# samuel-vitorino/sopro

Measured on NVIDIA H100. Metric: ar_frames_per_sec, higher is better.
Workload: dtype f32 math / bf16 weight storage

## Files before the change

### include/sopro_b200.h

```cpp
#ifndef SOPRO_B200_H_
#define SOPRO_B200_H_

#include <stddef.h>
#include <stdint.h>

#ifdef __cplusplus
extern "C" {
#endif

#define SOPRO_MAX_AR_LAYERS 16

enum sopro_status {
  SOPRO_OK = 0,
  SOPRO_ERR_INVALID = -1,
  SOPRO_ERR_CUDA = -2,
  SOPRO_ERR_UNSUPPORTED = -3,
  SOPRO_ERR_STATE = -4
};

enum sopro_wdtype { SOPRO_W_F32 = 0, SOPRO_W_BF16 = 1 };

typedef struct sopro_ar_config {
  int32_t d_model;
  int32_t n_layers;
// ... 64 lines not shown
int sopro_ar_session_create(sopro_engine_t* e, int max_batch, int max_steps, int max_text_len,
                            sopro_ar_session_t** out);
int sopro_ar_session_destroy(sopro_ar_session_t* s);

int sopro_ar_session_set_team(sopro_ar_session_t* s, int utts_per_team);

int sopro_ar_begin(sopro_ar_session_t* s, int batch, int steps, const float* cond_ar,
                   const float* txt_seq, int text_stride, const int32_t* text_len,
                   const float* noise, int noise_k, const sopro_ar_sampling_t* sampling,
                   void* stream);

int sopro_ar_run(sopro_ar_session_t* s, int n_steps, void* stream);

int sopro_ar_outputs(sopro_ar_session_t* s, const int32_t** tokens, const int32_t** n_tokens,
                     const int32_t** done);
int sopro_ar_read(sopro_ar_session_t* s, int32_t* tokens_host, int32_t* n_tokens_host,
                  int32_t* done_host, void* stream);
int sopro_ar_position(sopro_ar_session_t* s);

int sopro_ar_generate_host(sopro_ar_session_t* s, int batch, int steps, const float* cond_ar,
                           const float* txt_seq, int text_stride, const int32_t* text_len,
                           const float* noise, int noise_k, const sopro_ar_sampling_t* sampling,
                           int32_t* tokens_out, int32_t* n_tokens_out, void* stream);

typedef struct sopro_noise sopro_noise_t;
int sopro_noise_create(uint64_t seed, sopro_noise_t** out);
int sopro_noise_rows(sopro_noise_t* g, int n_rows, int vocab, int keep, float* out);
int sopro_noise_destroy(sopro_noise_t* g);

int sopro_ar_set_forced_tokens(sopro_ar_session_t* s, const int32_t* forced);
int sopro_ar_set_trace(sopro_ar_session_t* s, float* trace_blocks, float* trace_logits);
int sopro_ar_set_timing(sopro_ar_session_t* s, int64_t* buf, int step);
int sopro_ar_set_attn_trace(sopro_ar_session_t* s, float* probs, int64_t ld);
int sopro_ar_debug_sampled(sopro_ar_session_t* s, int32_t* dst, void* stream);
int sopro_ar_debug_kv(sopro_ar_session_t* s, float* k_dst, float* v_dst, void* stream);
int sopro_debug_pack_w6(const float* W, int N, int K, uint16_t* out);
int sopro_debug_sample(const float* logits, int vocab, const int32_t* hist, int n_hist, const float* noise, int noise_k,
                       const sopro_ar_sampling_t* sampling, int recovery, int device, int32_t* token_out);


#define SOPRO_MIMI_MAX_LAYERS 16
#define SOPRO_MIMI_MAX_RATIOS 8

typedef struct sopro_mimi_config {
  int32_t hidden;
  int32_t codebook_dim;
  int32_t n_q;
  int32_t n_sem;
  int32_t vocab;
  int32_t n_layers;
  int32_t n_heads;
  int32_t ffn;
  int32_t window;
  int32_t num_filters;
  int32_t kernel;
  int32_t last_kernel;
  int32_t res_kernel;
  int32_t compress;
  int32_t n_ratios;
  int32_t ratios[SOPRO_MIMI_MAX_RATIOS];
  float norm_eps;
  float rope_theta;
} sopro_mimi_config_t;

typedef struct sopro_mimi_layer_weights {
  const float *ln1_w, *ln1_b;
// ... 318 lines not shown
```

### sopro_b200/_lib.py

```python
from __future__ import annotations

import ctypes as C
import math
import os
from typing import List, Optional, Sequence

import torch

MAX_AR_LAYERS = 16
_HERE = os.path.dirname(os.path.abspath(__file__))
LIB_PATH = os.path.join(_HERE, "lib", "libsopro_b200.so")


class SoproError(RuntimeError):
    pass


class ArConfig(C.Structure):
    _fields_ = [
        ("d_model", C.c_int32), ("n_layers", C.c_int32), ("kernel", C.c_int32), ("n_heads", C.c_int32),
        ("vocab", C.c_int32), ("eos_id", C.c_int32),
        ("dilation", C.c_int32 * MAX_AR_LAYERS), ("has_attn", C.c_int32 * MAX_AR_LAYERS),
        ("weight_dtype", C.c_int32),
    ]
# ... 103 lines not shown

class RefPrepKvLayer(C.Structure):
    _fields_ = [(n, C.POINTER(C.c_float)) for n in ("nkv_w", "k_w", "v_w")]


class RefPrepWeights(C.Structure):
    _fields_ = [(n, C.POINTER(C.c_float)) for n in ("sv_emb", "sv_cb_weights", "sv_dw0_w", "sv_dw0_b", "sv_dw1_w", "sv_dw1_b",
                                                    "pool_w0", "pool_b0", "pool_w2")] + [("pool_b2", C.c_float)] + [
        (n, C.POINTER(C.c_float)) for n in ("proj_w", "proj_b", "cb_embed", "ref_cb_weights")] + [
        ("ref_block", SsmBlockWeights * 16), ("ref_norm_w", C.POINTER(C.c_float)), ("layer", RefPrepKvLayer * 8)]


_VP, _I, _I32P = C.c_void_p, C.c_int, C.POINTER(C.c_int32)
SYMBOLS = {
    "sopro_last_error": (C.c_char_p, []),
    "sopro_version": (C.c_char_p, []),
    "sopro_engine_create": (_I, [C.POINTER(ArConfig), C.POINTER(ArWeights), _I, C.POINTER(_VP)]),
    "sopro_engine_destroy": (_I, [_VP]),
    "sopro_engine_step_weight_bytes": (C.c_int64, [_VP]),
    "sopro_engine_num_sms": (_I, [_VP]),
    "sopro_ar_session_create": (_I, [_VP, _I, _I, _I, C.POINTER(_VP)]),
    "sopro_ar_session_destroy": (_I, [_VP]),
    "sopro_ar_session_set_team": (_I, [_VP, _I]),
    "sopro_ar_begin": (_I, [_VP, _I, _I, _VP, _VP, _I, _I32P, _VP, _I, C.POINTER(ArSampling), _VP]),
    "sopro_ar_run": (_I, [_VP, _I, _VP]),
    "sopro_ar_outputs": (_I, [_VP, C.POINTER(_VP), C.POINTER(_VP), C.POINTER(_VP)]),
    "sopro_ar_read": (_I, [_VP, _VP, _VP, _VP, _VP]),
    "sopro_ar_position": (_I, [_VP]),
    "sopro_ar_generate_host": (_I, [_VP, _I, _I, _VP, _VP, _I, _I32P, _VP, _I, C.POINTER(ArSampling), _VP, _VP, _VP]),
    "sopro_ar_set_forced_tokens": (_I, [_VP, _VP]),
    "sopro_ar_set_trace": (_I, [_VP, _VP, _VP]),
    "sopro_ar_set_timing": (_I, [_VP, _VP, _I]),
    "sopro_ar_set_attn_trace": (_I, [_VP, _VP, C.c_int64]),
    "sopro_ar_debug_sampled": (_I, [_VP, _VP, _VP]),
    "sopro_ar_debug_kv": (_I, [_VP, _VP, _VP, _VP]),
    "sopro_noise_create": (_I, [C.c_uint64, _VP]),
    "sopro_noise_rows": (_I, [_VP, _I, _I, _I, _VP]),
    "sopro_noise_destroy": (_I, [_VP]),
    "sopro_debug_pack_w6": (_I, [_VP, _I, _I, _VP]),
    "sopro_debug_sample": (_I, [_VP, _I, _VP, _I, _VP, _I, _VP, _I, _I, _VP]),
    "sopro_mimi_create": (_I, [C.POINTER(MimiConfigC), C.POINTER(MimiWeights), _I, C.POINTER(_VP)]),
    "sopro_mimi_destroy": (_I, [_VP]),
    "sopro_mimi_samples_per_frame": (C.c_int64, [_VP]),
    "sopro_mimi_decode": (_I, [_VP, _VP, _I, _I, _VP, _VP]),
    "sopro_mimi_decode_host": (_I, [_VP, _VP, _I, _I, _VP, _VP]),
    "sopro_mimi_set_precision": (_I, [_VP, _I]),
    "sopro_mimi_set_graphs": (_I, [_VP, _I]),
    "sopro_mimi_check": (_I, [_VP, _VP]),
    "sopro_mimi_stream_create": (_I, [_VP, _I, C.POINTER(_VP)]),
    "sopro_mimi_stream_destroy": (_I, [_VP]),
    "sopro_mimi_stream_reset": (_I, [_VP, _VP]),
    "sopro_mimi_stream_frames": (C.c_int64, [_VP]),
    "sopro_mimi_decode_step": (_I, [_VP, _VP, _I, _VP, _VP]),
    "sopro_mimi_decode_step_host": (_I, [_VP, _VP, _I, _VP, _VP]),
    "sopro_mimi_encoder_create": (_I, [C.POINTER(MimiConfigC), C.POINTER(MimiEncoderWeights), _I, C.POINTER(_VP)]),
    "sopro_mimi_encoder_destroy": (_I, [_VP]),
    "sopro_mimi_encoded_frames": (C.c_int64, [_VP, C.c_int64]),
    "sopro_mimi_encode": (_I, [_VP, _VP, C.c_int64, _VP, _VP, _VP]),
    "sopro_mimi_encode_host": (_I, [_VP, _VP, C.c_int64, _VP, _VP, _VP]),
    "sopro_nar_create": (_I, [_VP, _VP, _I, C.POINTER(_VP)]),
    "sopro_nar_destroy": (_I, [_VP]),
    "sopro_nar_set_forced": (_I, [_VP, _VP]),
    "sopro_nar_set_contraction": (_I, [_VP, _I]),
    "sopro_nar_set_graphs": (_I, [_VP, _I]),
    "sopro_nar_set_trace": (_I, [_VP, _VP]),
    "sopro_debug_dense": (_I, [_VP, _VP, _VP, _VP, _VP, _VP, _VP, C.c_float, _I, _I, _I, _I, _I, _I, C.c_int64, C.c_int64,
# ... 185 lines not shown
```

### sopro_b200/csrc/ar_engine.cu

```cuda
#include <cuda_runtime.h>

#include <algorithm>
#include <cstdio>
#include <cstring>
#include <string>
#include <vector>

#include "../../include/sopro_b200.h"
#include "common.cuh"
#include "ar_kernel.cuh"

using namespace sopro;

namespace {

thread_local std::string g_err;

size_t align_up(size_t x, size_t a) { return (x + a - 1) / a * a; }

uint16_t f32_to_bf16_rne(float f) {
  uint32_t u;
  memcpy(&u, &f, 4);
  if ((u & 0x7fffffffu) > 0x7f800000u) return (uint16_t)((u >> 16) | 0x40);
  const uint32_t lsb = (u >> 16) & 1u;
// ... 23 lines not shown
};

}

namespace mimi {
void set_error(const char* msg) { g_err = msg; }
}

struct sopro_engine {
  int device = 0;
  int n_sms = 0;
  sopro_ar_config_t cfg{};
  int D = 0, F = 0, V = 0, Vpad = 0, H = 0, Dh = 0, Kc = 0, n_layers = 0, n_attn = 0;
  unsigned char* dev = nullptr;
  size_t dev_bytes = 0;
  int64_t step_weight_bytes = 0;
  LayerDev layer[kMaxLayers]{};
  const float* nkv_w[kMaxLayers]{};
  const void* wk[kMaxLayers]{};
  const void* wv[kMaxLayers]{};
  const float* final_norm_w = nullptr;
  const void* head_w = nullptr;
  const float* head_b = nullptr;
  const float* emb = nullptr;
  const float* epi[kMaxLayers]{};
  int KcP = 0, KcE = 0;
  long long ring_floats_per_utt = 0;
};

struct sopro_ar_session {
  sopro_engine* e = nullptr;
  int max_batch = 0, max_steps = 0, Lmax = 0;
  int utts_per_team = 0;
  float *ring = nullptr, *xa = nullptr, *xb = nullptr, *hbuf = nullptr, *qbuf = nullptr, *abuf = nullptr,
        *logits = nullptr, *kc = nullptr, *vc = nullptr;
  int *tokens = nullptr, *sampled = nullptr, *text_len = nullptr, *n_tokens = nullptr, *done = nullptr;
  UttState* st = nullptr;
  SamplingDev* samp = nullptr;
  unsigned* barrier = nullptr;
  unsigned* tok_ll = nullptr;
  unsigned seq_base = 0;
  TileDesc* tiles = nullptr;
  int* n_tiles = nullptr;
  unsigned char* stage_tiles = nullptr;
  std::vector<unsigned char> h_stage_tiles;
  int tile_P = -1, tile_wbuf = -1, tile_qatt = -1;
  bool qatt = false;
  std::vector<TileDesc> h_tiles;
  std::vector<int> h_ntiles;
  float *h_cond = nullptr, *h_txt = nullptr, *h_noise = nullptr;
  size_t h_cond_cap = 0, h_txt_cap = 0, h_noise_cap = 0;
  int B = 0, steps = 0, noise_k = 0, t_pos = 0;
  const float* cond = nullptr;
  const float* noise = nullptr;
  const int* forced = nullptr;
  float* trace_blocks = nullptr;
  float* trace_logits = nullptr;
  long long* timing = nullptr;
  int timing_step = -1;
  float* attn_trace = nullptr;
  int64_t attn_ld = 0;
  int max_len = 0;
  bool begun = false;
  std::vector<UttState> host_st;
  unsigned char* pin = nullptr;
  size_t pin_bytes = 0;
// ... 246 lines not shown
  A((void**)&s->n_tokens, B * 4);
  A((void**)&s->done, B * 4);
  A((void**)&s->st, B * sizeof(UttState));
  A((void**)&s->samp, B * sizeof(SamplingDev));
  A((void**)&s->barrier, (size_t)e->n_sms * 32 * 4);
  A((void**)&s->tiles, (size_t)e->n_sms * kMaxTilesPerStep * sizeof(TileDesc));
  A((void**)&s->n_tiles, (size_t)e->n_sms * 4);
  A((void**)&s->stage_tiles, (size_t)e->n_sms * kMaxStages);
  if (err != cudaSuccess) {
    session_free(s);
    delete s;
    return fail(SOPRO_ERR_CUDA, "session allocation failed: %s", cudaGetErrorString(err));
  }
  *out = s;
  return SOPRO_OK;
}

int sopro_ar_session_destroy(sopro_ar_session_t* s) {
  if (!s) return SOPRO_OK;
  cudaSetDevice(s->e->device);
  session_free(s);
  delete s;
  return SOPRO_OK;
}

int sopro_ar_session_set_team(sopro_ar_session_t* s, int utts_per_team) {
  if (!s) return fail(SOPRO_ERR_INVALID, "null session");
  if (utts_per_team < 0 || utts_per_team > kMaxUttPerTeam)
    return fail(SOPRO_ERR_INVALID, "utts_per_team must be in [0,%d]", kMaxUttPerTeam);
  s->utts_per_team = utts_per_team;
  return SOPRO_OK;
}

}

template <typename WT>
static int launch_kv(sopro_ar_session* s, const float* txt, int text_stride, const std::vector<int>& lens,
                     cudaStream_t st) {
  sopro_engine* e = s->e;
  if (e->n_attn == 0) return SOPRO_OK;
  KvParams kp{};
  kp.D = e->D;
  kp.H = e->H;
  kp.Dh = e->Dh;
  kp.B = s->B;
  kp.Lmax = s->Lmax;
  kp.text_stride = text_stride;
  kp.n_attn = e->n_attn;
  kp.txt = txt;
  kp.text_len = s->text_len;
  for (int i = 0; i < e->n_attn; ++i) {
    kp.nkv_w[i] = e->nkv_w[i];
    kp.wk[i] = e->wk[i];
    kp.wv[i] = e->wv[i];
  }
  kp.kc = s->kc;
  kp.vc = s->vc;
  int maxlen = 0;
  for (int v : lens) maxlen = std::max(maxlen, v);
  dim3 grid((maxlen + 15) / 16, s->B, e->n_attn);
  const size_t smem = (size_t)16 * e->D * 4;
  CK(cudaFuncSetAttribute(kv_build_kernel<WT>, cudaFuncAttributeMaxDynamicSharedMemorySize, (int)smem));
  kv_build_kernel<WT><<<grid, kThreads, smem, st>>>(kp);
  CK(cudaGetLastError());
  return SOPRO_OK;
}
// ... 155 lines not shown
        t.src0 = reinterpret_cast<unsigned long long>(base + (size_t)a * row_bytes);
        t.bytes0 = (unsigned)((size_t)nr * row_bytes);
        t.src1 = sw.parts == 2 ? reinterpret_cast<unsigned long long>(base + (size_t)(a + sw.N) * row_bytes) : 0ull;
        t.bytes1 = sw.parts == 2 ? t.bytes0 : 0u;
        t.src2 = 0;
        t.bytes2 = 0;
        t.off2 = 0;
        if (sw.parts == 2) {
          t.src2 = reinterpret_cast<unsigned long long>(sw.epi + (size_t)a * e->KcE);
          t.bytes2 = (unsigned)((size_t)nr * e->KcE * 4);
        } else if (sw.epi) {
          const int lo = a / 4 * 4, hi = (a + nr + 3) / 4 * 4;
          t.src2 = reinterpret_cast<unsigned long long>(sw.epi + lo);
          t.bytes2 = (unsigned)((hi - lo) * 4);
          t.off2 = a - lo;
        }
        t.row0 = a;
        t.nrows = nr;
        if (++s->h_stage_tiles[(size_t)r * kMaxStages + sw.stage] == 255)
          return fail(SOPRO_ERR_INVALID, "more than 254 weight tiles in one stage");
      }
    }
    s->h_ntiles[r] = n;
  }
  CK(cudaMemcpyAsync(s->tiles, s->h_tiles.data(), s->h_tiles.size() * sizeof(TileDesc), cudaMemcpyHostToDevice, st));
  CK(cudaMemcpyAsync(s->n_tiles, s->h_ntiles.data(), (size_t)P * 4, cudaMemcpyHostToDevice, st));
  CK(cudaMemcpyAsync(s->stage_tiles, s->h_stage_tiles.data(), s->h_stage_tiles.size(), cudaMemcpyHostToDevice, st));
  s->tile_P = P;
  s->tile_wbuf = wbuf;
  s->tile_qatt = (int)qatt;
  return SOPRO_OK;
}

template <typename WT, int TU, bool LL>
static int launch_ar_tu(sopro_ar_session* s, ArParams& p, size_t smem, int grid, cudaStream_t st) {
  auto kern = p.attn_trace ? ar_persistent_kernel<WT, TU, LL, true> : ar_persistent_kernel<WT, TU, LL, false>;
  CK(cudaFuncSetAttribute(kern, cudaFuncAttributeMaxDynamicSharedMemorySize, (int)smem));
  int occ = 0;
  CK(cudaOccupancyMaxActiveBlocksPerMultiprocessor(&occ, kern, kThreads, smem));
  if (occ < 1) return fail(SOPRO_ERR_CUDA, "persistent kernel does not fit an SM (smem %zu)", smem);
  CK(cudaMemsetAsync(s->barrier, 0, (size_t)s->e->n_sms * 32 * 4, st));
  void* args[] = {(void*)&p};
  CK(cudaLaunchCooperativeKernel((const void*)kern, dim3(grid), dim3(kThreads), args, smem, st));
  s->seq_base += (unsigned)((p.t_end - p.t_begin) * p.n_stage);
  return SOPRO_OK;
}

template <typename WT>
static int launch_ar(sopro_ar_session* s, int t_begin, int t_end, cudaStream_t st) {
  sopro_engine* e = s->e;
  ArParams p{};
  p.D = e->D;
  p.F = e->F;
  p.V = e->V;
  p.Vpad = e->Vpad;
  p.H = e->H;
  p.Dh = e->Dh;
  p.Kc = e->Kc;
  p.KcP = e->KcP;
  p.KcE = e->KcE;
  p.n_layers = e->n_layers;
  p.eos_id = e->cfg.eos_id;
  long long roff = 0;
  for (int i = 0; i < e->n_layers; ++i) {
    p.layer[i] = e->layer[i];
    p.layer[i].ring_off = roff;
// ... 107 lines not shown
  p.PH = PH;
  s->qatt = qatt;
  int rc = build_tiles(s, P, (int)wbuf, st);
  if (rc != SOPRO_OK) return rc;
  p.tiles = s->tiles;
  p.n_tiles = s->n_tiles;
  p.stage_tiles = s->stage_tiles;
  p.nbuf = nbuf;
  p.wbuf_bytes = (int)wbuf;
  p.act_bytes = (int)act_bytes;
  p.ring_off = (int)act_bytes;
  p.table_off = (int)(act_bytes + (size_t)nbuf * wbuf);
  const size_t smem = act_bytes + (size_t)nbuf * wbuf + table_bytes + 1024;
  {
    int n = 0;
    for (int i = 0; i < e->n_layers; ++i) {
      p.prog[n++] = {K_GLU, (unsigned char)i};
      p.prog[n++] = {K_FFN1, (unsigned char)i};
      p.prog[n++] = {K_FFN2, (unsigned char)i};
      if (e->layer[i].has_attn) {
        if (qatt) {
          p.prog[n++] = {K_QATT, (unsigned char)i};
        } else {
          p.prog[n++] = {K_Q, (unsigned char)i};
          p.prog[n++] = {K_ATT, (unsigned char)i};
        }
        p.prog[n++] = {K_O, (unsigned char)i};
      }
    }
    p.prog[n++] = {K_HEAD, 0};
    p.prog[n++] = {K_SAMPLE, 0};
    p.n_stage = n;
  }
  const int grid = g * P;
  const char* sync_env = getenv("SOPRO_AR_SYNC");
  bool ll = Bt <= 8;
  if (sync_env && strcmp(sync_env, "barrier") == 0) ll = false;
  if (sync_env && strcmp(sync_env, "ll") == 0) ll = true;
  if (ll) {
    if (Bt >= 8) return launch_ar_tu<WT, 8, true>(s, p, smem, grid, st);
    if (Bt >= 4) return launch_ar_tu<WT, 4, true>(s, p, smem, grid, st);
    if (Bt >= 2) return launch_ar_tu<WT, 2, true>(s, p, smem, grid, st);
    return launch_ar_tu<WT, 1, true>(s, p, smem, grid, st);
  }
  if (Bt >= 8) return launch_ar_tu<WT, 8, false>(s, p, smem, grid, st);
  if (Bt >= 4) return launch_ar_tu<WT, 4, false>(s, p, smem, grid, st);
  if (Bt >= 2) return launch_ar_tu<WT, 2, false>(s, p, smem, grid, st);
  return launch_ar_tu<WT, 1, false>(s, p, smem, grid, st);
}

extern "C" {

int sopro_ar_run(sopro_ar_session_t* s, int n_steps, void* stream) {
  if (!s) return fail(SOPRO_ERR_INVALID, "null session");
  if (!s->begun) return fail(SOPRO_ERR_STATE, "sopro_ar_run before sopro_ar_begin");
  if (n_steps < 1) return fail(SOPRO_ERR_INVALID, "n_steps must be >= 1");
  sopro_engine* e = s->e;
  CK(cudaSetDevice(e->device));
  const int t0 = s->t_pos;
  const int t1 = std::min(s->steps, t0 + n_steps);
  if (t0 >= t1) return SOPRO_OK;
  if (s->attn_trace && s->attn_ld < s->max_len)
    return fail(SOPRO_ERR_INVALID, "attention trace row stride %lld < longest text %d", (long long)s->attn_ld, s->max_len);
  cudaStream_t st = reinterpret_cast<cudaStream_t>(stream);
  int rc = e->cfg.weight_dtype == SOPRO_W_F32 ? launch_ar<float>(s, t0, t1, st)
                                               : launch_ar<__nv_bfloat16>(s, t0, t1, st);
  if (rc != SOPRO_OK) return rc;
  s->t_pos = t1;
  return SOPRO_OK;
}

int sopro_ar_outputs(sopro_ar_session_t* s, const int32_t** tokens, const int32_t** n_tokens,
                     const int32_t** done) {
  if (!s) return fail(SOPRO_ERR_INVALID, "null session");
  if (tokens) *tokens = s->tokens;
  if (n_tokens) *n_tokens = s->n_tokens;
  if (done) *done = s->done;
  return SOPRO_OK;
}

// ... 188 lines not shown
```

### sopro_b200/csrc/ar_kernel.cuh

```cuda
#pragma once
#include <cuda_bf16.h>
#include <cuda_runtime.h>
#include <stdint.h>

namespace sopro {

constexpr int kThreads = 512;
constexpr int kWarps = kThreads / 32;
constexpr int kMaxLayers = 16;
constexpr int kMaxTopK = 64;
constexpr int kCand = 128;
constexpr int kMaxUttPerTeam = 32;
constexpr int kMaxVocab = 8 * kThreads;
constexpr int kTapSlots = 16;
constexpr int kTimingSlots = 224;
constexpr int kMaxStages = 6 * kMaxLayers + 2;
constexpr int kMaxTilesPerStep = 128;
constexpr int kMaxWBuf = 8;

__device__ __forceinline__ float2 ffma2(float2 a, float2 b, float2 c) { return make_float2(fmaf(a.x, b.x, c.x), fmaf(a.y, b.y, c.y)); }

enum StageKind { K_GLU = 0, K_FFN1 = 1, K_FFN2 = 2, K_Q = 3, K_O = 4, K_HEAD = 5, K_ATT = 6, K_SAMPLE = 7, K_QATT = 8 };

struct LayerDev {
  const float* norm_w;
  const void* glu_w;
  const float* glu_b;
  const float* dw_w;
  const float* dw_b;
  const float* ffn_norm_w;
  const void* w1;
  const float* b1;
  const void* w2;
  const float* b2;
  const float* nq_w;
  const void* wq;
  const void* wo;
  float gate_tanh;
  int has_attn;
  int attn_slot;
  int dil;
  int ring_len;
  long long ring_off;
};

struct UttState {
  int len;
  int last;
  int streak;
  int recovery;
  int done;
  int pad[3];
};

struct SamplingDev {
  float top_p, temperature, rec_top_p, rec_temp, rep_pen;
  int top_k, anti_loop, loop_streak, min_gen, stop_on_first_eos;
};

struct TileDesc {
  unsigned long long src0;
  unsigned long long src1;
  unsigned long long src2;
  unsigned bytes0, bytes1, bytes2;
  int off2;
  int row0;
  int nrows;
  int pad[4];
};
static_assert(sizeof(TileDesc) == 64, "the weight ring is sized around an 8 KB tile table");

struct StageOp {
  unsigned char kind, layer;
};

struct ArParams {
  int D, F, V, Vpad, H, Dh, Kc, KcP, KcE, n_layers, eos_id;
  LayerDev layer[kMaxLayers];
  StageOp prog[kMaxStages];
  int n_stage;
  const float* final_norm_w;
  const void* head_w;
  const float* head_b;
  const float* emb;
  int B, steps, Lmax, noise_k;
  const float* cond;
  const float* noise;
  const float* kc;
  const float* vc;
  const int* text_len;
  float* ring;
  float* xa;
  float* xb;
  float* hbuf;
  float* qbuf;
  float* abuf;
  float* logits;
  int* tokens;
  int* sampled;
  int* n_tokens;
  int* done;
  const int* forced;
  UttState* st;
  const SamplingDev* samp;
  float* trace_blocks;
  float* trace_logits;
// ... 236 lines not shown
      --inflight;
    }
  }
};

template <int N>
__device__ __forceinline__ float reduce_transposed(float (&v)[N], int lane) {
  int n = N;
#pragma unroll
  for (int s = 16; s >= 1; s >>= 1) {
    if (n > 1) {
      const int half = n >> 1;
      const bool up = (lane & s) != 0;
#pragma unroll
      for (int i = 0; i < N / 2; ++i) {
        if (i < half) {
          const float keep = up ? v[i + half] : v[i];
          const float send = up ? v[i] : v[i + half];
          v[i] = keep + __shfl_xor_sync(0xffffffffu, send, s);
        }
      }
      n = half;
    } else {
      v[0] += __shfl_xor_sync(0xffffffffu, v[0], s);
    }
  }
  return v[0];
}
template <>
__device__ __forceinline__ float reduce_transposed<1>(float (&v)[1], int lane) {
  return warp_sum(v[0]);
}

template <int R, int TU, typename WT>
__device__ __forceinline__ float warp_rows_s(const unsigned (&w)[R], unsigned act, int K, int lane) {
  float2 acc[R][TU];
#pragma unroll
  for (int r = 0; r < R; ++r)
#pragma unroll
    for (int u = 0; u < TU; ++u) acc[r][u] = make_float2(0.f, 0.f);
#pragma unroll(R * TU >= 32 ? 1 : 3)
  for (int k = lane * 4; k < K; k += 128) {
    float4 wv[R];
#pragma unroll
    for (int r = 0; r < R; ++r) wv[r] = ldsw4<WT>(w[r] + (unsigned)k * (unsigned)sizeof(WT));
#pragma unroll
    for (int u = 0; u < TU; ++u) {
      const float4 x = lds128(act + ((unsigned)u * (unsigned)K + (unsigned)k) * 4u);
#pragma unroll
      for (int r = 0; r < R; ++r) {
        acc[r][u] = ffma2(make_float2(wv[r].x, wv[r].y), make_float2(x.x, x.y), acc[r][u]);
        acc[r][u] = ffma2(make_float2(wv[r].z, wv[r].w), make_float2(x.z, x.w), acc[r][u]);
      }
    }
  }
  float v[R * TU];
#pragma unroll
  for (int r = 0; r < R; ++r)
#pragma unroll
    for (int u = 0; u < TU; ++u) v[r * TU + u] = acc[r][u].x + acc[r][u].y;
  return reduce_transposed<R * TU>(v, lane);
}

template <int TU, typename WT>
__device__ __forceinline__ void warp_rows_g(const WT* w0, const WT* w1, const float* __restrict__ act, int K, int lane,
                                            float (&out)[2][TU]) {
  float2 acc[2][TU];
#pragma unroll
  for (int u = 0; u < TU; ++u) acc[0][u] = acc[1][u] = make_float2(0.f, 0.f);
#pragma unroll 3
  for (int k = lane * 4; k < K; k += 128) {
    const float4 wa = ldw4(w0 + k);
    const float4 wb = ldw4(w1 + k);
#pragma unroll
// ... 817 lines not shown
    for (int j = grp; j < n_my; j += 2) {
      const int u = gi + j * PH;
      attention_item<TRACE>(p, L, tc.b0 + u, h, qh + (size_t)j * Dh, sc, part, grp, gt, LL ? 1 : 0, out_seq);
    }
  }
}

template <typename WT, int TU, bool LL, bool TRACE = false>
__global__ void __launch_bounds__(kThreads, 1) ar_persistent_kernel(const __grid_constant__ ArParams p) {
  extern __shared__ __align__(128) unsigned char smem_raw[];
  __shared__ SamplerSmem ssm;
  __shared__ __align__(8) unsigned long long wbars[kMaxWBuf];
  __shared__ unsigned char stage_tiles[kMaxStages];
  __shared__ int conv_phase[kMaxLayers], conv_slot[kMaxLayers];
  __shared__ int s_tok[kMaxUttPerTeam], s_done[kMaxUttPerTeam];
  constexpr int EL = LL ? 2 : 1;
  unsigned char* const smem_base = smem_raw + ((1024u - (smem_u32(smem_raw) & 1023u)) & 1023u);
  float* act = reinterpret_cast<float*>(smem_base);
  TeamCtx tc;
  tc.team = blockIdx.x / p.P;
  tc.rank = blockIdx.x % p.P;
  tc.P = p.P;
  if (tc.team >= p.g) return;
  tc.b0 = tc.team * p.Bt;
  tc.nb = min(p.Bt, p.B - tc.b0);
  if (tc.nb <= 0) return;
  const int warp = threadIdx.x >> 5, lane = threadIdx.x & 31;
  unsigned* bar = p.barrier + (size_t)tc.team * 32;
  unsigned epoch = 0;
  const int D = p.D, F = p.F;
  const unsigned act_s = smem_u32(act);
  float* xraw = act + (size_t)tc.nb * D;
  const unsigned scratch_s = act_s + (unsigned)(2 * tc.nb * D) * 4u;
  const int n_ut = (tc.nb + TU - 1) / TU;
  WeightRing ring;
  {
    TileDesc* tab = reinterpret_cast<TileDesc*>(smem_base + p.table_off);
    const int nt = p.n_tiles[tc.rank];
    const TileDesc* gt = p.tiles + (size_t)tc.rank * kMaxTilesPerStep;
    for (int i = threadIdx.x; i < nt; i += kThreads) tab[i] = gt[i];
    for (int i = threadIdx.x; i < p.n_stage; i += kThreads) stage_tiles[i] = p.stage_tiles[(size_t)tc.rank * kMaxStages + i];
    if (threadIdx.x == 0) {
      for (int i = 0; i < p.nbuf; ++i) mbar_init(&wbars[i], 1);
      asm volatile("fence.mbarrier_init.release.cluster;" ::: "memory");
    }
    __syncthreads();
    ring.bars = wbars;
    ring.base = smem_u32(smem_base + p.ring_off);
    ring.wbuf = (unsigned)p.wbuf_bytes;
    ring.nbuf = p.nbuf;
    ring.table = tab;
    ring.n_tiles = nt;
    ring.start((p.t_end - p.t_begin) * nt);
  }

#pragma unroll 1
  for (int t = p.t_begin; t < p.t_end; ++t) {
    const unsigned seq0 = p.seq_base + (unsigned)((t - p.t_begin) * p.n_stage);
    if (threadIdx.x < tc.nb) {
      const int b = tc.b0 + threadIdx.x;
      int tok = 0, dn = 0;
      if (LL && t > p.t_begin) {
        uint2 w;
        do {
          w = ll_load1(reinterpret_cast<const float*>(p.tok_ll) + (size_t)b * 2);
        } while (w.y != seq0);
        tok = (int)(w.x & 0x3fffffffu);
// ... 68 lines not shown
        }
        if (src == nullptr) {
          for (int u = warp; u < tc.nb; u += kWarps) {
            const int b = tc.b0 + u;
            const float* cr = p.cond + ((size_t)b * p.steps + t) * D;
            for (int k = lane * 4; k < D; k += 128) cp_async16(act_s + (unsigned)(u * D + k) * 4u, cr + k);
            const int row = (t == 0) ? p.V : s_tok[u];
            const float* er = p.emb + (size_t)row * D;
            for (int k = lane * 4; k < D; k += 128) cp_async16(act_s + (unsigned)((tc.nb + u) * D + k) * 4u, er + k);
          }
          cp_async_commit();
          cp_async_wait0();
          __syncwarp();
          for (int u = warp; u < tc.nb; u += kWarps) {
            for (int k = lane * 4; k < D; k += 128) {
              const float4 c = *reinterpret_cast<float4*>(act + (size_t)u * D + k);
              const float4 e = *reinterpret_cast<float4*>(xraw + (size_t)u * D + k);
              const float4 x = make_float4(c.x + e.x, c.y + e.y, c.z + e.z, c.w + e.w);
              *reinterpret_cast<float4*>(act + (size_t)u * D + k) = x;
              *reinterpret_cast<float4*>(xraw + (size_t)u * D + k) = x;
            }
          }
          __syncwarp();
        }
        stage_rows<LL>(src ? src + (size_t)tc.b0 * K * EL : nullptr, tc.nb, K, act, norm_w,
                       (kind == K_GLU && src) ? xraw : nullptr, src_seq);
        __syncthreads();
        ts.mark();
        const bool glu = kind == K_GLU;
        const unsigned row_bytes = (unsigned)K * (unsigned)sizeof(WT);
        float* state = p.ring + L.ring_off;
        const int dil = L.dil;
        const int phase = conv_phase[li], slot_now = conv_slot[li];
#pragma unroll 1
      for (int ti = stage_tiles[si]; ti > 0; --ti) {
        const TileDesc* td;
        const unsigned wb = ring.acquire(td);
        const int nr = td->nrows;
        constexpr int R = (TU == 8) ? 4 : 2;
        constexpr int RC = R / 2;
        const int n_rt = glu ? (nr + RC - 1) / RC : (nr + R - 1) / R;
        const unsigned epi_s = wb + td->bytes0 + td->bytes1;
#pragma unroll 1
        for (int task = warp; task < n_rt * n_ut; task += kWarps) {
          const int rt = n_ut == 1 ? task : (int)((unsigned)task / (unsigned)n_ut);
          const int u0 = (task - rt * n_ut) * TU;
          unsigned wr[R];
#pragma unroll
          for (int jr = 0; jr < R; ++jr) {
            if (glu) {
              const int ch = min(rt * RC + (jr % RC), nr - 1);
              wr[jr] = wb + (jr < RC ? 0u : td->bytes0) + (unsigned)ch * row_bytes;
            } else {
              wr[jr] = wb + (unsigned)min(rt * R + jr, nr - 1) * row_bytes;
            }
          }
          const int ub = min(u0, max(tc.nb - TU, 0));
          constexpr int NOUT = R * TU;
          constexpr int LOG2N = (NOUT == 2 ? 1 : NOUT == 4 ? 2 : NOUT == 8 ? 3 : NOUT == 16 ? 4 : 5);
          constexpr int SH = 5 - LOG2N;
          const int o = (lane >> SH) & (NOUT - 1);
          const int i = o / TU, uu = o % TU;
          const bool writer = (lane & ((1 << SH) - 1)) == 0;
          const int ri = glu ? rt * RC + i : rt * R + i;
          const int u = ub + uu;
          const bool mine = writer && (glu ? i < RC : true) && ri < nr && u >= u0 && u < tc.nb;
          const int r = td->row0 + ri;
          const int b = tc.b0 + (mine ? u : 0);
          float* d = dst + ((size_t)b * ld_dst + (mine ? r : td->row0)) * EL;
          float res_v = 0.f;
          float* rb = nullptr;
          const unsigned tap_w = scratch_s + (unsigned)warp * (unsigned)(kTapSlots * p.KcP * 4) +
                                 (unsigned)((i % RC) * TU + uu) * (unsigned)(p.KcP * 4);
          if (glu) {
            rb = state + (((size_t)b * D + (mine ? r : td->row0)) * dil + phase) * p.KcP;
            if (mine)
              for (int q = 0; q < p.KcP; q += 4) cp_async16(tap_w + (unsigned)q * 4u, rb + q);
          } else if (mine && (kind == K_FFN2 || kind == K_O)) {
            res_v = ldcg1(d);
          }
          cp_async_commit();
          float v = warp_rows_s<R, TU, WT>(wr, act_s + (unsigned)ub * (unsigned)K * 4u, K, lane);
          const float gate_v = __shfl_sync(0xffffffffu, v, (((RC + (i % RC)) * TU + uu) << SH) & 31);
          cp_async_wait0();
          if (mine) {
            if (glu) {
              const int Kc = p.Kc;
              const unsigned er = epi_s + (unsigned)(ri * p.KcE) * 4u;
              const float a = v + lds32(er + (unsigned)(Kc + 1) * 4u);
              const float gt = gate_v + lds32(er + (unsigned)(Kc + 2) * 4u);
              const float h = a * sigmoid_ref(gt);
              rb[slot_now] = h;
              float y = 0.f;
              int pos = slot_now + 1;
#pragma unroll 1
              for (int j = 0; j < Kc - 1; ++j) {
                if (pos == Kc) pos = 0;
                y += lds32(tap_w + (unsigned)pos * 4u) * lds32(er + (unsigned)j * 4u);
                ++pos;
              }
              y += h * lds32(er + (unsigned)(Kc - 1) * 4u);
              y += lds32(er + (unsigned)Kc * 4u);
              v = xraw[(size_t)u * D + r] + y;
            } else {
              const float bias_v = (kind == K_Q || kind == K_O) ? 0.f : lds32(epi_s + (unsigned)(td->off2 + ri) * 4u);
              if (kind == K_FFN1) {
                v = gelu_erf(v + bias_v);
              } else if (kind == K_FFN2) {
                v = res_v + (v + bias_v);
                if (trace) trace[(size_t)b * D + r] = v;
              } else if (kind == K_O) {
                v = res_v + scale * v;
                if (trace) trace[(size_t)b * D + r] = v;
              } else if (kind == K_HEAD) {
                v += bias_v;
                if (trace) trace[(size_t)b * p.V + r] = v;
// ... 96 lines not shown
```

### sopro_b200/engine.py

```python
from __future__ import annotations

import ctypes as C
import dataclasses
from typing import Dict, List, Optional, Sequence, Union

import numpy as np
import torch

from . import _lib
from .config import SoproTTSConfig


@dataclasses.dataclass
class Sampling:
    top_p: float = 0.9
    temperature: float = 1.05
    recovery_top_p: float = 0.85
    recovery_temp: float = 1.2
    repetition_penalty: float = 1.1
    top_k: int = 50
    anti_loop: bool = True
    loop_streak: int = 8
    min_gen_frames: int = 12
    stop_on_first_eos: bool = False
# ... 154 lines not shown
        n = np.zeros((B,), dtype=np.int32)
        _lib.check(self.lib.sopro_ar_generate_host(
            self._h, B, steps, pc, pt, int(stx[1]), lens, pn, int(sn[2]), arr, toks.ctypes.data, n.ctypes.data,
            _lib.stream_ptr(self.engine.device)))
        self.batch, self.steps = B, steps
        return toks, n

    def set_forced(self, forced: Optional[torch.Tensor]) -> None:
        if forced is None:
            _lib.check(self.lib.sopro_ar_set_forced_tokens(self._h, None))
            return
        f = forced.to(device=self.engine.device, dtype=torch.int32).contiguous()
        self._forced = f
        _lib.check(self.lib.sopro_ar_set_forced_tokens(self._h, f.data_ptr()))

    def set_trace(self, blocks: Optional[torch.Tensor], logits: Optional[torch.Tensor]) -> None:
        self._trace = (blocks, logits)
        _lib.check(self.lib.sopro_ar_set_trace(self._h, blocks.data_ptr() if blocks is not None else None,
                                               logits.data_ptr() if logits is not None else None))

    def set_attn_trace(self, probs: Optional[torch.Tensor]) -> None:
        if probs is None:
            self._attn_trace = None
            _lib.check(self.lib.sopro_ar_set_attn_trace(self._h, None, 0))
            return
        assert probs.dtype == torch.float32 and probs.is_contiguous() and probs.device == self.engine.device and probs.dim() == 5
        self._attn_trace = probs
        _lib.check(self.lib.sopro_ar_set_attn_trace(self._h, probs.data_ptr(), int(probs.shape[-1])))

    def set_timing(self, buf: Optional[torch.Tensor], step: int = -1) -> None:
        self._timing = buf
        _lib.check(self.lib.sopro_ar_set_timing(self._h, buf.data_ptr() if buf is not None else None, int(step)))

    def sampled(self) -> torch.Tensor:
        out = torch.empty((self.batch, self.steps), dtype=torch.int32, device=self.engine.device)
        _lib.check(self.lib.sopro_ar_debug_sampled(self._h, out.data_ptr(), _lib.stream_ptr(self.engine.device)))
        return out

    def kv(self):
        cfg = self.engine.cfg
        n_attn = len(cfg.ar_attn_layers())
        Lp = (self.max_text_len + 3) // 4 * 4
        shape = (n_attn, self.batch, cfg.AR_HEADS, Lp, int(cfg.d_model) // cfg.AR_HEADS)
        ko = torch.empty(shape, dtype=torch.float32, device=self.engine.device)
        vo = torch.empty(shape, dtype=torch.float32, device=self.engine.device)
        _lib.check(self.lib.sopro_ar_debug_kv(self._h, ko.data_ptr(), vo.data_ptr(), _lib.stream_ptr(self.engine.device)))
        return ko, vo

    def close(self) -> None:
        if getattr(self, "_h", None):
            self.lib.sopro_ar_session_destroy(self._h)
            self._h = None

    def __del__(self):
        try:
            self.close()
        except Exception:
            pass
```

Before: 325,900.

## Add per-stage narrow task shape for GEMV stages chosen by host load model

Adds a per-stage task shape (wide or narrow) for GEMV stages in the persistent AR kernel. In narrow mode each warp task covers half as many utterances, giving more tasks per tile. A host-side cost model estimates the worst per-partition load under both shapes and picks narrow when it looks clearly cheaper, with an override API for forcing either mode. This aims to balance warps across tiles for small batches, at the cost of more runtime shape logic, a second template instantiation of the inner product, and more activation reads per weight row.

```diff
diff --git a/include/sopro_b200.h b/include/sopro_b200.h
--- a/include/sopro_b200.h
+++ b/include/sopro_b200.h
@@ -120,6 +120,8 @@
 int sopro_ar_set_trace(sopro_ar_session_t* s, float* trace_blocks, float* trace_logits);
 int sopro_ar_set_timing(sopro_ar_session_t* s, int64_t* buf, int step);
 int sopro_ar_set_attn_trace(sopro_ar_session_t* s, float* probs, int64_t ld);
+int sopro_ar_session_set_task_shape(sopro_ar_session_t* s, int mode);
+int sopro_ar_session_stage_shapes(sopro_ar_session_t* s, int32_t* kinds, int32_t* shapes, int cap, int32_t* n_stage);
 int sopro_ar_debug_sampled(sopro_ar_session_t* s, int32_t* dst, void* stream);
 int sopro_ar_debug_kv(sopro_ar_session_t* s, float* k_dst, float* v_dst, void* stream);
 int sopro_debug_pack_w6(const float* W, int N, int K, uint16_t* out);
diff --git a/sopro_b200/_lib.py b/sopro_b200/_lib.py
--- a/sopro_b200/_lib.py
+++ b/sopro_b200/_lib.py
@@ -159,6 +159,8 @@
     "sopro_ar_set_trace": (_I, [_VP, _VP, _VP]),
     "sopro_ar_set_timing": (_I, [_VP, _VP, _I]),
     "sopro_ar_set_attn_trace": (_I, [_VP, _VP, C.c_int64]),
+    "sopro_ar_session_set_task_shape": (_I, [_VP, _I]),
+    "sopro_ar_session_stage_shapes": (_I, [_VP, _I32P, _I32P, _I, _I32P]),
     "sopro_ar_debug_sampled": (_I, [_VP, _VP, _VP]),
     "sopro_ar_debug_kv": (_I, [_VP, _VP, _VP, _VP]),
     "sopro_noise_create": (_I, [C.c_uint64, _VP]),
diff --git a/sopro_b200/csrc/ar_engine.cu b/sopro_b200/csrc/ar_engine.cu
--- a/sopro_b200/csrc/ar_engine.cu
+++ b/sopro_b200/csrc/ar_engine.cu
@@ -79,6 +79,9 @@
   sopro_engine* e = nullptr;
   int max_batch = 0, max_steps = 0, Lmax = 0;
   int utts_per_team = 0;
+  int task_shape = 0;
+  StageOp last_prog[kMaxStages]{};
+  int last_n_stage = 0;
   float *ring = nullptr, *xa = nullptr, *xb = nullptr, *hbuf = nullptr, *qbuf = nullptr, *abuf = nullptr,
         *logits = nullptr, *kc = nullptr, *vc = nullptr;
   int *tokens = nullptr, *sampled = nullptr, *text_len = nullptr, *n_tokens = nullptr, *done = nullptr;
@@ -391,6 +394,24 @@
   return SOPRO_OK;
 }
 
+int sopro_ar_session_set_task_shape(sopro_ar_session_t* s, int mode) {
+  if (!s) return fail(SOPRO_ERR_INVALID, "null session");
+  if (mode < 0 || mode > 2) return fail(SOPRO_ERR_INVALID, "task shape mode must be 0 (auto), 1 (wide) or 2 (narrow)");
+  s->task_shape = mode;
+  return SOPRO_OK;
+}
+
+int sopro_ar_session_stage_shapes(sopro_ar_session_t* s, int32_t* kinds, int32_t* shapes, int cap, int32_t* n_stage) {
+  if (!s) return fail(SOPRO_ERR_INVALID, "null session");
+  if (cap < 0 || (cap > 0 && (!kinds || !shapes))) return fail(SOPRO_ERR_INVALID, "stage_shapes: bad output buffers");
+  for (int i = 0; i < s->last_n_stage && i < cap; ++i) {
+    kinds[i] = s->last_prog[i].kind;
+    shapes[i] = s->last_prog[i].shape;
+  }
+  if (n_stage) *n_stage = s->last_n_stage;
+  return SOPRO_OK;
+}
+
 }
 
 template <typename WT>
@@ -612,6 +633,38 @@
   return SOPRO_OK;
 }
 
+static void pick_task_shapes(sopro_ar_session* s, ArParams& p, int P, int TU, int Bt) {
+  const int R = TU == 8 ? 4 : 2, RC = R / 2;
+  std::vector<int> first(P, 0);
+  for (int si = 0; si < p.n_stage; ++si) {
+    StageOp& op = p.prog[si];
+    op.shape = SHAPE_WIDE;
+    const bool gemv = op.kind <= K_HEAD;
+    const int K = op.kind == K_FFN2 ? s->e->F : s->e->D;
+    long long load[2] = {0, 0};
+    for (int r = 0; r < P; ++r) {
+      const int nt = s->h_stage_tiles[(size_t)r * kMaxStages + si];
+      long long l[2] = {0, 0};
+      for (int j = 0; gemv && j < nt; ++j) {
+        const int nr = s->h_tiles[(size_t)r * kMaxTilesPerStep + first[r] + j].nrows;
+        const int n_rt = op.kind == K_GLU ? (nr + RC - 1) / RC : (nr + R - 1) / R;
+        for (int w = 0; w < 2; ++w) {
+          const int tue = w ? std::max(TU / 2, 1) : TU;
+          const long long tasks = (long long)n_rt * ((Bt + tue - 1) / tue);
+          l[w] += (tasks + 3) / 4 * R * tue * K;
+        }
+      }
+      first[r] += nt;
+      load[0] = std::max(load[0], l[0]);
+      load[1] = std::max(load[1], l[1]);
+    }
+    if (!gemv || TU < 2 || op.kind == K_GLU) continue;
+    if (s->task_shape == 2 || (s->task_shape == 0 && 6 * load[1] < 5 * load[0])) op.shape = SHAPE_NARROW;
+  }
+  std::copy(p.prog, p.prog + p.n_stage, s->last_prog);
+  s->last_n_stage = p.n_stage;
+}
+
 template <typename WT, int TU, bool LL>
 static int launch_ar_tu(sopro_ar_session* s, ArParams& p, size_t smem, int grid, cudaStream_t st) {
   auto kern = p.attn_trace ? ar_persistent_kernel<WT, TU, LL, true> : ar_persistent_kernel<WT, TU, LL, false>;
@@ -785,20 +838,22 @@
     p.prog[n++] = {K_SAMPLE, 0};
     p.n_stage = n;
   }
+  const int TU = Bt >= 8 ? 8 : Bt >= 4 ? 4 : Bt >= 2 ? 2 : 1;
+  pick_task_shapes(s, p, P, TU, Bt);
   const int grid = g * P;
   const char* sync_env = getenv("SOPRO_AR_SYNC");
   bool ll = Bt <= 8;
   if (sync_env && strcmp(sync_env, "barrier") == 0) ll = false;
   if (sync_env && strcmp(sync_env, "ll") == 0) ll = true;
   if (ll) {
-    if (Bt >= 8) return launch_ar_tu<WT, 8, true>(s, p, smem, grid, st);
-    if (Bt >= 4) return launch_ar_tu<WT, 4, true>(s, p, smem, grid, st);
-    if (Bt >= 2) return launch_ar_tu<WT, 2, true>(s, p, smem, grid, st);
+    if (TU == 8) return launch_ar_tu<WT, 8, true>(s, p, smem, grid, st);
+    if (TU == 4) return launch_ar_tu<WT, 4, true>(s, p, smem, grid, st);
+    if (TU == 2) return launch_ar_tu<WT, 2, true>(s, p, smem, grid, st);
     return launch_ar_tu<WT, 1, true>(s, p, smem, grid, st);
   }
-  if (Bt >= 8) return launch_ar_tu<WT, 8, false>(s, p, smem, grid, st);
-  if (Bt >= 4) return launch_ar_tu<WT, 4, false>(s, p, smem, grid, st);
-  if (Bt >= 2) return launch_ar_tu<WT, 2, false>(s, p, smem, grid, st);
+  if (TU == 8) return launch_ar_tu<WT, 8, false>(s, p, smem, grid, st);
+  if (TU == 4) return launch_ar_tu<WT, 4, false>(s, p, smem, grid, st);
+  if (TU == 2) return launch_ar_tu<WT, 2, false>(s, p, smem, grid, st);
   return launch_ar_tu<WT, 1, false>(s, p, smem, grid, st);
 }
 
diff --git a/sopro_b200/csrc/ar_kernel.cuh b/sopro_b200/csrc/ar_kernel.cuh
--- a/sopro_b200/csrc/ar_kernel.cuh
+++ b/sopro_b200/csrc/ar_kernel.cuh
@@ -17,6 +17,8 @@
 constexpr int kMaxStages = 6 * kMaxLayers + 2;
 constexpr int kMaxTilesPerStep = 128;
 constexpr int kMaxWBuf = 8;
+
+__host__ __device__ constexpr int ilog2(int n) { return n > 1 ? 1 + ilog2(n / 2) : 0; }
 
 __device__ __forceinline__ float2 ffma2(float2 a, float2 b, float2 c) { return make_float2(fmaf(a.x, b.x, c.x), fmaf(a.y, b.y, c.y)); }
 
@@ -70,8 +72,10 @@
 };
 static_assert(sizeof(TileDesc) == 64, "the weight ring is sized around an 8 KB tile table");
 
+enum TaskShape { SHAPE_WIDE = 0, SHAPE_NARROW = 1 };
+
 struct StageOp {
-  unsigned char kind, layer;
+  unsigned char kind, layer, shape;
 };
 
 struct ArParams {
@@ -374,14 +378,14 @@
   return warp_sum(v[0]);
 }
 
-template <int R, int TU, typename WT>
+template <int R, int TU, typename WT, int UNROLL = (R * TU >= 32 ? 1 : 3)>
 __device__ __forceinline__ float warp_rows_s(const unsigned (&w)[R], unsigned act, int K, int lane) {
   float2 acc[R][TU];
 #pragma unroll
   for (int r = 0; r < R; ++r)
 #pragma unroll
     for (int u = 0; u < TU; ++u) acc[r][u] = make_float2(0.f, 0.f);
-#pragma unroll(R * TU >= 32 ? 1 : 3)
+#pragma unroll(UNROLL)
   for (int k = lane * 4; k < K; k += 128) {
     float4 wv[R];
 #pragma unroll
@@ -1265,7 +1269,6 @@
   const unsigned act_s = smem_u32(act);
   float* xraw = act + (size_t)tc.nb * D;
   const unsigned scratch_s = act_s + (unsigned)(2 * tc.nb * D) * 4u;
-  const int n_ut = (tc.nb + TU - 1) / TU;
   WeightRing ring;
   {
     TileDesc* tab = reinterpret_cast<TileDesc*>(smem_base + p.table_off);
@@ -1400,19 +1403,25 @@
         float* state = p.ring + L.ring_off;
         const int dil = L.dil;
         const int phase = conv_phase[li], slot_now = conv_slot[li];
+        constexpr int R = (TU == 8) ? 4 : 2;
+        constexpr int RC = R / 2;
+        constexpr int TUN = TU >= 2 ? TU / 2 : TU;
+        const bool narrow = TUN != TU && p.prog[si].shape == SHAPE_NARROW;
+        const int lg_tue = narrow ? ilog2(TUN) : ilog2(TU);
+        const int tue = 1 << lg_tue;
+        const int sh = 5 - ilog2(R) - lg_tue;
+        const int n_ut = (tc.nb + tue - 1) >> lg_tue;
 #pragma unroll 1
       for (int ti = stage_tiles[si]; ti > 0; --ti) {
         const TileDesc* td;
         const unsigned wb = ring.acquire(td);
         const int nr = td->nrows;
-        constexpr int R = (TU == 8) ? 4 : 2;
-        constexpr int RC = R / 2;
         const int n_rt = glu ? (nr + RC - 1) / RC : (nr + R - 1) / R;
         const unsigned epi_s = wb + td->bytes0 + td->bytes1;
 #pragma unroll 1
         for (int task = warp; task < n_rt * n_ut; task += kWarps) {
           const int rt = n_ut == 1 ? task : (int)((unsigned)task / (unsigned)n_ut);
-          const int u0 = (task - rt * n_ut) * TU;
+          const int u0 = (task - rt * n_ut) << lg_tue;
           unsigned wr[R];
 #pragma unroll
           for (int jr = 0; jr < R; ++jr) {
@@ -1423,13 +1432,10 @@
               wr[jr] = wb + (unsigned)min(rt * R + jr, nr - 1) * row_bytes;
             }
           }
-          const int ub = min(u0, max(tc.nb - TU, 0));
-          constexpr int NOUT = R * TU;
-          constexpr int LOG2N = (NOUT == 2 ? 1 : NOUT == 4 ? 2 : NOUT == 8 ? 3 : NOUT == 16 ? 4 : 5);
-          constexpr int SH = 5 - LOG2N;
-          const int o = (lane >> SH) & (NOUT - 1);
-          const int i = o / TU, uu = o % TU;
-          const bool writer = (lane & ((1 << SH) - 1)) == 0;
+          const int ub = min(u0, max(tc.nb - tue, 0));
+          const int o = (lane >> sh) & ((R << lg_tue) - 1);
+          const int i = o >> lg_tue, uu = o & (tue - 1);
+          const bool writer = (lane & ((1 << sh) - 1)) == 0;
           const int ri = glu ? rt * RC + i : rt * R + i;
           const int u = ub + uu;
           const bool mine = writer && (glu ? i < RC : true) && ri < nr && u >= u0 && u < tc.nb;
@@ -1439,7 +1445,7 @@
           float res_v = 0.f;
           float* rb = nullptr;
           const unsigned tap_w = scratch_s + (unsigned)warp * (unsigned)(kTapSlots * p.KcP * 4) +
-                                 (unsigned)((i % RC) * TU + uu) * (unsigned)(p.KcP * 4);
+                                 (unsigned)((i % RC) * tue + uu) * (unsigned)(p.KcP * 4);
           if (glu) {
             rb = state + (((size_t)b * D + (mine ? r : td->row0)) * dil + phase) * p.KcP;
             if (mine)
@@ -1448,8 +1454,9 @@
             res_v = ldcg1(d);
           }
           cp_async_commit();
-          float v = warp_rows_s<R, TU, WT>(wr, act_s + (unsigned)ub * (unsigned)K * 4u, K, lane);
-          const float gate_v = __shfl_sync(0xffffffffu, v, (((RC + (i % RC)) * TU + uu) << SH) & 31);
+          const unsigned xa = act_s + (unsigned)ub * (unsigned)K * 4u;
+          float v = narrow ? warp_rows_s<R, TUN, WT, 1>(wr, xa, K, lane) : warp_rows_s<R, TU, WT>(wr, xa, K, lane);
+          const float gate_v = __shfl_sync(0xffffffffu, v, (((RC + (i % RC)) * tue + uu) << sh) & 31);
           cp_async_wait0();
           if (mine) {
             if (glu) {
diff --git a/sopro_b200/engine.py b/sopro_b200/engine.py
--- a/sopro_b200/engine.py
+++ b/sopro_b200/engine.py
@@ -210,6 +210,16 @@
         self._timing = buf
         _lib.check(self.lib.sopro_ar_set_timing(self._h, buf.data_ptr() if buf is not None else None, int(step)))
 
+    STAGE_KINDS = ("glu", "ffn1", "ffn2", "q", "o", "head", "att", "sample", "qatt")
+
+    def set_task_shape(self, mode: int) -> None:
+        _lib.check(self.lib.sopro_ar_session_set_task_shape(self._h, int(mode)))
+
+    def stage_shapes(self):
+        kinds, shapes, n = (C.c_int32 * 128)(), (C.c_int32 * 128)(), C.c_int32()
+        _lib.check(self.lib.sopro_ar_session_stage_shapes(self._h, kinds, shapes, 128, C.byref(n)))
+        return [(self.STAGE_KINDS[kinds[i]], ("wide", "narrow")[shapes[i]]) for i in range(n.value)]
+
     def sampled(self) -> torch.Tensor:
         out = torch.empty((self.batch, self.steps), dtype=torch.int32, device=self.engine.device)
         _lib.check(self.lib.sopro_ar_debug_sampled(self._h, out.data_ptr(), _lib.stream_ptr(self.engine.device)))
```

New measurement: 340,600, median of 6. 1.05x the previous value.
